# vaibhawvipul/taper

Hardware: AMD Instinct MI355X
Metric: MNIST samples/sec fwd+bwd+step (higher is better)
Workload: dtype f32; 1 GPU; mlp_784-128-10_b64; per_gpu_batch=64, global_batch=64, parallelism=single, comm=none, graph_record_steps=11577

## Files before the change

### include/taper_hip_debug.h

```cpp
#ifndef TAPER_HIP_DEBUG_H
#define TAPER_HIP_DEBUG_H

#include "taper_hip.h"

#ifdef __cplusplus
extern "C" {
#endif

int th_debug_mlp3_calls(int64_t *out);
int th_debug_mlp2_calls(int64_t *out);
int th_debug_mlp2_only(int which);
int th_debug_mlp2_ksplit(int ksplit);
int th_debug_set_chain_loop(int on);
int th_debug_chain_mlp3_only(int which);
int th_debug_set_chain_generic(int on);
int th_debug_last_conv_config(th_ctx *ctx, int *out6);
int th_debug_set_conv_img(th_ctx *ctx, int mode);
int th_debug_conv3x3_plan(int op, int n, int c_in, int h, int w, int c_out, int pad, int weight_layout, int relu_bias, int accumulate,
                          int w_misalign_bytes, int img_mode, int *out32);
int th_debug_qlinear_plan(int qtype, int batch, int in_features, int out_features, int x_misalign_bytes, int w_misalign_bytes, int *out8);
int th_debug_q8q8_plan(int batch, int in_features, int out_features, int *out4);
int th_debug_qconv_plan(int n, int c_in, int h, int w, int c_out, int k_h, int k_w, int s_h, int s_w, int pad_h, int pad_w, int *out8);
int th_debug_sgemm_plan(int trans_a, int trans_b, int m, int n, int k, int a_misalign_bytes, int b_misalign_bytes, int c_misalign_bytes, int *out12);
int th_debug_linear_fwd_ex_plan(int batch, int in_features, int out_features, int subtiles, int *out8);

int th_comm_debug_dump(th_comm *comm, th_ctx *ctx);
#ifdef __cplusplus
}
#endif

#endif
```

### taper_amd/csrc/common.h

```cpp
#pragma once

#include <hip/hip_runtime.h>

#include <cstdarg>
#include <cstdint>
#include <cstdio>
#include <array>
#include <atomic>
#include <map>
#include <string>
#include <unordered_map>
#include <unordered_set>
#include <vector>

#include "../../include/taper_hip.h"
#include "../../include/taper_hip_debug.h"

namespace th {

void set_error(const char *fmt, ...);

#define TH_HIP(expr)                                                                         \
    do {                                                                                     \
        hipError_t e_ = (expr);                                                              \
        if (e_ != hipSuccess) {                                                              \
            th::set_error("%s failed: %s (%s:%d)", #expr, hipGetErrorString(e_), __FILE__, __LINE__); \
            return 1;                                                                        \
        }                                                                                    \
    } while (0)

#define TH_REQUIRE(cond, ...)              \
    do {                                   \
        if (!(cond)) {                     \
            th::set_error(__VA_ARGS__);    \
            return 2;                      \
        }                                  \
    } while (0)

#define TH_SET_MAX_LDS(ctx_, fn_, bytes_)                                                                                \
    do {                                                                                                                 \
        static std::atomic<unsigned long long> th_lds_done_{0ull};                                                       \
        static std::atomic<int> th_lds_max_{0};                                                                          \
        const unsigned long long th_lds_bit_ = 1ull << ((ctx_)->device & 63);                                            \
        const int th_lds_want_ = (int)(bytes_);                                                                          \
        if (!(th_lds_done_.load(std::memory_order_relaxed) & th_lds_bit_) || th_lds_want_ > th_lds_max_.load(std::memory_order_relaxed)) { \
            TH_HIP(hipFuncSetAttribute((const void *)(fn_), hipFuncAttributeMaxDynamicSharedMemorySize, th_lds_want_));  \
            int th_lds_prev_ = th_lds_max_.load(std::memory_order_relaxed);                                              \
            if (th_lds_want_ > th_lds_prev_) {                                                                           \
                th_lds_max_.store(th_lds_want_, std::memory_order_relaxed);                                              \
                th_lds_done_.store(th_lds_bit_, std::memory_order_relaxed);    \
            } else {                                                                                                     \
                th_lds_done_.fetch_or(th_lds_bit_, std::memory_order_relaxed);                                           \
            }                                                                                                            \
        }                                                                                                                \
    } while (0)

#define TH_LAUNCH_CHECK() TH_HIP(hipGetLastError())

constexpr int kWave = 64;
constexpr int kNumCU = 256;
constexpr int kNumXCD = 8;

static inline int ceil_div(long a, long b) { return (int)((a + b - 1) / b); }

__device__ __forceinline__ void lds_barrier() {
    __builtin_amdgcn_fence(__ATOMIC_RELEASE, "workgroup", "local");
    __builtin_amdgcn_s_barrier();
    __builtin_amdgcn_fence(__ATOMIC_ACQUIRE, "workgroup", "local");
}

enum : int32_t { TH_DEVERR_NONE = 0, TH_DEVERR_TARGET_OOB = 1 };
static __device__ __attribute__((unused)) int32_t *g_err_word;
__device__ __forceinline__ void raise_target_oob(long cls, int classes) {
    int32_t *w = g_err_word;
    if (!w) return;
    w[1] = (int32_t)(cls > 0x7fffffffL ? 0x7fffffffL : cls);
    w[2] = classes;
    __threadfence_system();
    w[0] = TH_DEVERR_TARGET_OOB;
}
typedef int (*err_bind_fn)(int32_t *);
struct ErrBindReg { explicit ErrBindReg(err_bind_fn f); };
#define TH_USES_DEVICE_ERRORS()                                                                                        \
    namespace {                                                                                                        \
    int th_err_bind_here(int32_t *p) { return hipMemcpyToSymbol(HIP_SYMBOL(th::g_err_word), &p, sizeof(p)) == hipSuccess ? 0 : 1; } \
    th::ErrBindReg th_err_reg_here(th_err_bind_here);                                                                  \
    }

static inline int ew_grid(size_t n_items, int block) {
    long g = (long)((n_items + block - 1) / block);
    long cap = (long)kNumCU * 8;
    return (int)(g < 1 ? 1 : (g > cap ? cap : g));
}

}

struct th_ctx {
    int device = 0;
    hipStream_t stream = nullptr;
    std::multimap<size_t, void *> free_blocks;
    std::unordered_map<void *, size_t> block_size;
    std::unordered_set<void *> graph_owned;
    std::unordered_set<void *> graph_owned_freed;
    size_t bytes_reserved = 0, bytes_in_use = 0;
    bool capturing = false;
    std::vector<void *> capture_blocks;
    std::multimap<size_t, void *> capture_free;
    std::map<std::array<int, 8>, void *> conv_plans;
    int32_t *err_word = nullptr;
    int m2_max_ksplit = 8;
    bool fwd_subtiles = true;
    bool tail_split = true;
    const uint32_t *update_guard = nullptr;
    uint32_t *update_step_word = nullptr;
    unsigned *m2_arrive = nullptr;
};

struct th_graph {
    th_ctx *ctx = nullptr;
    hipGraph_t graph = nullptr;
    hipGraphExec_t exec = nullptr;
    std::vector<void *> blocks;
};

struct th_event {
    hipEvent_t ev = nullptr;
};
```

### taper_amd/csrc/fwd_tick.hip

```cpp
#include "small16_dev.h"

namespace th {

constexpr int kFwdAVec = 1, kFwdBVec = 2, kFwdXcd = 4;

struct FwdTickRest {
    float *C;
    const float *bias;
    int relu;
    int32_t *tick;
    AdamSlices x;
};

template <int NW, int RM, int RN>
__global__ __launch_bounds__(64 * NW) void sgemm_small16_tick(const float *X, const float *W, int m, int n, int k, int tile_rows, int grid_x,
                                                              int flags, FwdTickRest r) {
#ifdef TH_PROFILE
    __builtin_amdgcn_sched_barrier(0);
    const long long t_entry = wall_clock64();
    __builtin_amdgcn_sched_barrier(0);
#endif
    __shared__ float red[NW][64][4];
    if ((int)blockIdx.y < tile_rows) {
        int tm = blockIdx.y, tn = blockIdx.x;
        const int b = blockIdx.x + grid_x * blockIdx.y;
        if (flags & kFwdXcd) {
            constexpr int SBM = 32 / RM, SBN = 32 / RN;
            static_assert(SBN == 2 || SBN == 4, "sub-tiles of 16 or 8 columns");
            const int q = b & 7, j = b >> 3;
            tm = SBM * (q >> 2) + (j >> (SBN == 4 ? 2 : 1));
            tn = SBN * (q & 3) + (j & (SBN - 1));
        }
        const SmallArgs p{X, nullptr, W, r.C, nullptr, m, n, k, k, 1, 1, k, (k + 15) / 16 * 16, flags & kFwdAVec, flags & kFwdBVec,
                          Epilogue{1.0f, 0.0f, r.bias, r.relu, AdamDev{nullptr, nullptr, nullptr, nullptr, nullptr, 0.f, 0.f, 0.f, 0.f}, nullptr, nullptr}};
#ifdef TH_PROFILE
        small16_body<true, true, NW, false, RM, RN, true, true>(p, tm, tn, 0, red, t_entry, b);
#else
        small16_body<true, true, NW, false, RM, RN, false, true>(p, tm, tn, 0, red);
#endif
        return;
    }
    if (blockIdx.x == 0) adam_slices_then_tick(r.x, r.tick);
}

int fwd_tick_launch(th_ctx *ctx, const FwdTickLaunch &q, const float *d_x, const float *d_w, const float *d_b, float *d_y, int m, int n, int k,
                    int relu, const AdamSlices &x, int32_t *d_tick) {
    const FwdTickRest r{d_y, d_b, relu, d_tick, x};
    const int flags = (q.a_vec ? kFwdAVec : 0) | (q.b_vec ? kFwdBVec : 0) | (q.xcd_blocks ? kFwdXcd : 0);
    const dim3 grid(q.grid_x, q.grid_y, 1);
    const int tile_rows = q.grid_y - 1;
    if (q.rm == 8) hipLaunchKernelGGL((sgemm_small16_tick<16, 8, 8>), grid, dim3(1024), 0, ctx->stream, d_x, d_w, m, n, k, tile_rows, q.grid_x, flags, r);
    else if (q.waves == 16) hipLaunchKernelGGL((sgemm_small16_tick<16, 16, 16>), grid, dim3(1024), 0, ctx->stream, d_x, d_w, m, n, k, tile_rows, q.grid_x, flags, r);
    else hipLaunchKernelGGL((sgemm_small16_tick<4, 16, 16>), grid, dim3(256), 0, ctx->stream, d_x, d_w, m, n, k, tile_rows, q.grid_x, flags, r);
    TH_LAUNCH_CHECK();
    return 0;
}

}

#ifdef TH_PROFILE
extern "C" int th_debug_fwd_prof(th_ctx *ctx, long long *h_out, int n_blocks) {
    TH_REQUIRE(ctx && h_out && n_blocks >= 1 && n_blocks <= th::kFwdProfBlocks, "th_debug_fwd_prof: bad argument");
    TH_HIP(hipStreamSynchronize(ctx->stream));
    TH_HIP(hipMemcpyFromSymbol(h_out, HIP_SYMBOL(th::g_fwd_prof), (size_t)n_blocks * 2 * th::kFwdProfStamps * sizeof(long long)));
    return 0;
}
#endif
```

### taper_amd/csrc/gemm.hip

```cpp
#include "small16_dev.h"
#include "step_log_dev.h"

namespace th {

typedef float floatx16 __attribute__((ext_vector_type(16)));

static inline Epilogue make_ep(float alpha, float beta, const float *bias = nullptr, int relu = 0) {
    return Epilogue{alpha, beta, bias, relu, AdamDev{nullptr, nullptr, nullptr, nullptr, nullptr, 0.f, 0.f, 0.f, 0.f}, nullptr, nullptr};
}

__device__ __forceinline__ float epilogue_apply(float acc, float c_old, const Epilogue &ep, int col) {
    float v = ep.alpha * acc;
    if (ep.beta != 0.0f) v += ep.beta * c_old;
    if (ep.bias) v += ep.bias[col];
    if (ep.relu) v = v > 0.0f ? v : 0.0f;
    return v;
}

template <bool A_KC, bool B_KC, int NW>
__global__ __launch_bounds__(64 * NW) void sgemm_small16(SmallArgs p) {
    __shared__ float red[NW][64][4];
    small16_body<A_KC, B_KC, NW, false>(p, blockIdx.y, blockIdx.x, blockIdx.z, red);
}

// ... 749 lines not shown
    const long tiles = (long)pl.tiles_m * pl.tiles_n;
    pl.a_vec = a_kc && (a_bits & 15) == 0 && (a_rs % 4 == 0);
    pl.b_vec = b_kc && (b_bits & 15) == 0 && (b_cs % 4 == 0);
    int kz = 1;
    pl.waves = (tiles < 256 && k >= 256) ? 16 : 4;
    if (tiles < 64 && k >= 2048) {
        kz = (int)((256 + tiles - 1) / tiles);
        const int kz_max = k / 512;
        if (kz > kz_max) kz = kz_max;
        if (kz < 1) kz = 1;
    }
    if (k == 0) {
        pl.kslice = 16;
        pl.kz = 1;
        return;
    }
    int kslice = ceil_div(k, kz);
    kslice = (kslice + 15) / 16 * 16;
    pl.kslice = kslice;
    pl.kz = ceil_div(k, kslice);
}

static void plan_tile(GemmPlan &pl, int ts, int m, int n, int k, bool a_kc, bool b_kc, long lda, long ldb, uintptr_t a_bits, uintptr_t b_bits) {
    pl.tile = ts;
    pl.waves = 4;
    pl.tiles_m = ceil_div(m, ts);
    pl.tiles_n = ceil_div(n, ts);
    const int kz = ts == 128 ? tile128_kz(m, n, k) : tile64_kz(m, n, k);
    pl.kslice = ceil_div(ceil_div(k, kz), BK) * BK;
    pl.kz = ceil_div(k, pl.kslice);
    const bool vec = (a_bits & 15) == 0 && (b_bits & 15) == 0 && (lda % 4 == 0) && (ldb % 4 == 0) && ((a_kc ? k : m) % 4 == 0) &&
                     ((b_kc ? k : n) % 4 == 0) && m >= 4 && n >= 4 && k >= 4;
    const bool exact = (m % ts == 0) && (n % ts == 0) && (k % BK == 0) && vec && lda < (1L << 22) && ldb < (1L << 22);
    pl.a_vec = pl.b_vec = vec;
    pl.form = exact ? kFormExactDma : rag_dma(ts, a_kc, b_kc, k, vec, lda, ldb) ? kFormRagDma : vec ? kFormGuardVec : kFormGuardScalar;
    constexpr int kSliceXcdChunks = 14;
    pl.slice_xcd = pl.kz > 1 && pl.kslice >= kSliceXcdChunks * BK;
}

static GemmPlan gemm_plan(int trans_a, int trans_b, int m, int n, int k, uintptr_t a_bits, uintptr_t b_bits, uintptr_t c_bits) {
    const long a_rs = trans_a ? 1 : k, a_cs = trans_a ? m : 1;
    const long b_rs = trans_b ? 1 : n, b_cs = trans_b ? k : 1;
    const bool a_kc = !trans_a, b_kc = trans_b != 0;
    GemmPlan pl{};
    const TileClass tc = gemm_tile_class(m, n, k);
    if (tc == TileClass::Small) plan_small(pl, m, n, k, a_kc, b_kc, a_rs, b_cs, a_bits, b_bits);
    else plan_tile(pl, tc == TileClass::Tile128 ? 128 : 64, m, n, k, a_kc, b_kc, a_kc ? a_rs : a_cs, b_kc ? b_cs : b_rs, a_bits, b_bits);
    pl.reduce = pl.kz <= 1 ? kReduceNone : reduce_c_quad((long)m * n, c_bits) ? kReduceQuad : kReduceScalar;
    return pl;
}

int gemm_dispatch(th_ctx *ctx, int trans_a, int trans_b, int m, int n, int k, const float *A, const float *B, float *C,
                  const Epilogue &ep) {
    if (m == 0 || n == 0) return 0;
    const long a_rs = trans_a ? 1 : k, a_cs = trans_a ? m : 1;
    const long b_rs = trans_b ? 1 : n, b_cs = trans_b ? k : 1;
    const bool a_kc = !trans_a, b_kc = trans_b != 0;
    const GemmPlan pl = gemm_plan(trans_a, trans_b, m, n, k, (uintptr_t)A, (uintptr_t)B, (uintptr_t)C);
#define TH_GEMM_CASE(AK, BKC)                                                                         \
    if (a_kc == AK && b_kc == BKC)                                                                          \
        return pl.tile == 64  ? launch_tile<64, AK, BKC>(ctx, pl, A, B, C, m, n, k, a_rs, a_cs, b_rs, b_cs, ep) \
             : pl.tile == 128 ? launch_tile128<AK, BKC>(ctx, pl, A, B, C, m, n, k, a_rs, a_cs, b_rs, b_cs, ep)  \
                              : launch_small<AK, BKC>(ctx, pl, A, B, C, m, n, k, a_rs, a_cs, b_rs, b_cs, ep);
    TH_GEMM_CASE(true, true)
    TH_GEMM_CASE(true, false)
    TH_GEMM_CASE(false, true)
    TH_GEMM_CASE(false, false)
#undef TH_GEMM_CASE
    return 3;
}

int mlp3_grads_launch(th_ctx *ctx, const float *const dz[3], const float *const act[3], float *const dw[3], float *const db[3],
                      const int out_f[3], const int in_f[3], const th_adam_fuse *const wf[3], const th_adam_fuse *const bf[3], int batch,
                      const float *part, int n_blk, float *loss, float *ncorrect, float *metrics, int64_t capacity, int64_t *state,
                      int64_t advance, const float *gap_dx, const th_mlp3_gap *gap) {
    Mlp3GradArgs a{};
    int blocks = 0;
    for (int l = 0; l < 3; ++l) {
        LinearBwdArgs &q = a.job[l];
        const int tm = ceil_div(out_f[l], 16), tn = ceil_div(in_f[l], 16);
        q.dw_kz = 1;
        q.dw_tiles = dw[l] ? tm * tn : 0;
        q.n_dw = (q.dw_tiles + 7) & ~7;
        q.dw_tiles_m = tm;
        q.dw = SmallArgs{dz[l], nullptr, act[l], dw[l], nullptr, out_f[l], in_f[l], batch, 1, out_f[l], in_f[l], 1, (batch + 15) / 16 * 16, 0, 0,
                         make_ep(1.0f, 0.0f)};
        q.dw.ep.adam = make_adam_dev(dw[l] ? wf[l] : nullptr);
        q.db_adam = make_adam_dev(db[l] ? bf[l] : nullptr);
        q.dy = dz[l];
        q.db = db[l];
        q.batch = batch;
        q.out_f = out_f[l];
        q.n_db = db[l] ? ceil_div(out_f[l], 64) : 0;
        a.first[l] = blocks;
        blocks += q.n_dw + q.n_db;
    }
    a.first[3] = blocks;
    if (gap && gap->d_cnt) {
        a.gap_dx = gap_dx; a.gap_cnt = gap->d_cnt; a.gap_db = gap->d_gb; a.gap_c = in_f[0]; a.gap_hw = gap->hw;
        a.gap_adam = make_adam_dev(gap->b_fuse);
        blocks += ceil_div(a.gap_c, 16);
    }
    a.first[4] = blocks;
    a.part = part; a.n_blk = n_blk; a.batch = batch;
    a.loss = loss; a.ncorrect = ncorrect; a.metrics = metrics; a.capacity = capacity; a.state = state; a.advance = advance;
    hipLaunchKernelGGL(mlp3_grads_kernel, dim3(blocks + 1), dim3(256), 0, ctx->stream, a);
    TH_LAUNCH_CHECK();
    return 0;
}

int linear_fwd_partials(th_ctx *ctx, const float *x, const float *w, int m, int n, int k, float **partial_out, int *kz_out) {
    const int tiles_m = ceil_div(m, 16), tiles_n = ceil_div(n, 16);
    const long tiles = (long)tiles_m * tiles_n;
    SmallArgs p{x, nullptr, w, nullptr, nullptr, m, n, k, k, 1, 1, k, 0, 0, 0, make_ep(1.0f, 0.0f)};
    p.a_vec = aligned16(x) && (k % 4 == 0);
    p.b_vec = aligned16(w) && (k % 4 == 0);
    int kz = (int)std::min<long>((256 + tiles - 1) / tiles, k / 512);
    if (kz < 1) kz = 1;
    if (kz > 8) kz = 8;
    const int kslice = (ceil_div(k, kz) + 15) / 16 * 16;
    kz = ceil_div(k, kslice);
    p.kslice = kslice;
    void *ws = nullptr;
    if (th_malloc(ctx, (size_t)kz * m * n * sizeof(float), &ws)) return 1;
    p.partial = (float *)ws;
    if (tiles < 256 && k >= 256) hipLaunchKernelGGL((sgemm_small16<true, true, 16>), dim3(tiles_n, tiles_m, kz), dim3(1024), 0, ctx->stream, p);
    else hipLaunchKernelGGL((sgemm_small16<true, true, 4>), dim3(tiles_n, tiles_m, kz), dim3(256), 0, ctx->stream, p);
    TH_LAUNCH_CHECK();
    *partial_out = p.partial;
    *kz_out = kz;
    return 0;
}

struct FwdExPlan {
    int one_launch;
    int rm, rn;
    int waves;
    int grid_x, grid_y;
    int xcd_blocks;
};
static FwdExPlan fwd_ex_plan(int m, int n, int k, bool subtiles) {
    FwdExPlan pl{};
    const long tiles = (long)ceil_div(m, 16) * ceil_div(n, 16);
    if (!(m > 0 && n > 0 && k > 0 && !gemm_is_big(m, n, k) && !(tiles < 64 && k >= 2048))) return pl;
    pl.one_launch = 1;
    pl.rm = pl.rn = 16;
    pl.waves = (tiles < 256 && k >= 256) ? 16 : 4;
    if (subtiles && pl.waves == 16 && k <= 1024 && m <= 64 && n <= 128) pl.rm = pl.rn = 8;
    pl.grid_x = ceil_div(n, pl.rn);
    pl.grid_y = ceil_div(m, pl.rm) + 1;
    pl.xcd_blocks = pl.grid_x == 128 / pl.rn && pl.grid_y == 64 / pl.rm + 1;
    return pl;
}

}

using namespace th;

extern "C" {

#ifdef TH_PROFILE
int th_debug_gemm_prof(th_ctx *ctx, long long *h_out4) {
    TH_HIP(hipStreamSynchronize(ctx->stream));
    TH_HIP(hipMemcpyFromSymbol(h_out4, HIP_SYMBOL(th::g_gemm_prof), 4 * sizeof(long long)));
    return 0;
}
#endif

int th_sgemm(th_ctx *ctx, int trans_a, int trans_b, int m, int n, int k, float alpha, const float *d_a,
             const float *d_b, float beta, float *d_c) {
    TH_REQUIRE(ctx, "th_sgemm: null ctx");
    TH_REQUIRE(m >= 0 && n >= 0 && k >= 0, "th_sgemm: negative dimension");
    TH_REQUIRE((m == 0 || n == 0) || (d_c && (k == 0 || (d_a && d_b))), "th_sgemm: null device pointer");
    Epilogue ep = make_ep(alpha, beta);
    return gemm_dispatch(ctx, trans_a, trans_b, m, n, k, d_a, d_b, d_c, ep);
}

int th_debug_sgemm_plan(int trans_a, int trans_b, int m, int n, int k, int a_misalign_bytes, int b_misalign_bytes, int c_misalign_bytes, int *out12) {
    TH_REQUIRE(out12, "th_debug_sgemm_plan: null argument");
    TH_REQUIRE(m >= 1 && n >= 1 && k >= 0, "th_debug_sgemm_plan: bad shape m=%d n=%d k=%d", m, n, k);
    TH_REQUIRE(((a_misalign_bytes | b_misalign_bytes | c_misalign_bytes) & ~12) == 0,
               "th_debug_sgemm_plan: a float pointer lies 0, 4, 8 or 12 bytes off a 16-byte boundary (got %d %d %d)", a_misalign_bytes,
               b_misalign_bytes, c_misalign_bytes);
    const GemmPlan p = gemm_plan(trans_a != 0, trans_b != 0, m, n, k, (uintptr_t)a_misalign_bytes, (uintptr_t)b_misalign_bytes, (uintptr_t)c_misalign_bytes);
    const long wgs = (long)p.tiles_m * p.tiles_n * p.kz;
    const int out[12] = {p.tile, p.form, p.waves, p.a_vec, p.b_vec, p.kz, p.kslice, (int)std::min<long>(wgs, 0x7fffffff), p.slice_xcd, p.reduce,
                         p.tiles_m, p.tiles_n};
    std::copy(out, out + 12, out12);
    return 0;
}

int th_linear_fwd(th_ctx *ctx, const float *d_x, const float *d_w, const float *d_b, float *d_y, int batch,
                  int in_features, int out_features, int relu) {
    TH_REQUIRE(ctx && d_x && d_w && d_y, "th_linear_fwd: null argument");
    Epilogue ep = make_ep(1.0f, 0.0f, d_b, relu);
    return gemm_dispatch(ctx, 0, 1, batch, out_features, in_features, d_x, d_w, d_y, ep);
}

int th_linear_fwd_ex(th_ctx *ctx, const float *d_x, const float *d_w, const float *d_b, float *d_y, int batch, int in_features,
                     int out_features, int relu, const th_adam_slice *extra, int n_extra, int32_t *d_tick) {
    TH_REQUIRE(ctx && d_x && d_w && d_y, "th_linear_fwd_ex: null argument");
    TH_REQUIRE(n_extra >= 0 && n_extra <= TH_MAX_ADAM_SLICES && (n_extra == 0 || extra), "th_linear_fwd_ex: bad extra slices");
    for (int i = 0; i < n_extra; ++i)
        TH_REQUIRE(extra[i].f.d_p != d_w && extra[i].f.d_p != d_b, "th_linear_fwd_ex: a carried slice must not alias what this launch reads");
    const int m = batch, n = out_features, k = in_features;
    const FwdExPlan pl = fwd_ex_plan(m, n, k, ctx->fwd_subtiles != 0);
    if (pl.one_launch) {
        const FwdTickLaunch q{pl.rm, pl.waves, pl.grid_x, pl.grid_y, pl.xcd_blocks, aligned16(d_x) && (k % 4 == 0), aligned16(d_w) && (k % 4 == 0)};
        return fwd_tick_launch(ctx, q, d_x, d_w, d_b, d_y, m, n, k, relu, make_adam_slices(extra, n_extra, ctx), d_tick);
    }
    if (int rc = th_adam_slices(ctx, extra, n_extra)) return rc;
    if (d_tick)
        if (int rc = th_adam_tick(ctx, d_tick)) return rc;
    return th_linear_fwd(ctx, d_x, d_w, d_b, d_y, batch, in_features, out_features, relu);
}

int th_linear_fwd_ex_set_subtiles(th_ctx *ctx, int on) {
    TH_REQUIRE(ctx, "th_linear_fwd_ex_set_subtiles: null ctx");
    ctx->fwd_subtiles = on != 0;
    return 0;
}

int th_debug_linear_fwd_ex_plan(int batch, int in_features, int out_features, int subtiles, int *out8) {
    TH_REQUIRE(out8, "th_debug_linear_fwd_ex_plan: null argument");
    TH_REQUIRE(batch >= 1 && in_features >= 1 && out_features >= 1, "th_debug_linear_fwd_ex_plan: bad shape batch=%d in=%d out=%d", batch,
               in_features, out_features);
    const FwdExPlan pl = fwd_ex_plan(batch, out_features, in_features, subtiles != 0);
    const int out[8] = {pl.one_launch, pl.rm, pl.rn, pl.waves, 1, pl.grid_x, pl.grid_y, pl.xcd_blocks};
    std::copy(out, out + 8, out8);
    return 0;
}

}

namespace th {

constexpr int THIN_ROWS = 32;
__global__ __launch_bounds__(256) void linear_dx_thin_kernel(const float *__restrict__ dz, const float *__restrict__ w, const float *__restrict__ xmask,
                                                             float *__restrict__ dx, float *__restrict__ colpart, int batch, int in_f, int out_f,
                                                             int accumulate) {
    __shared__ float dzs[THIN_ROWS][16];
    const int t = threadIdx.x, r0 = blockIdx.y * THIN_ROWS, col = (blockIdx.x * 256 + t) * 4;
    for (int i = t; i < THIN_ROWS * 16; i += 256) {
        const int r = i >> 4, o = i & 15;
        dzs[r][o] = (r0 + r < batch && o < out_f) ? dz[(long)(r0 + r) * out_f + o] : 0.f;
    }
    float4 wv[16];
#pragma unroll
    for (int o = 0; o < 16; ++o) wv[o] = (o < out_f && col < in_f) ? *reinterpret_cast<const float4 *>(w + (long)o * in_f + col) : make_float4(0.f, 0.f, 0.f, 0.f);
    __syncthreads();
    if (col >= in_f) return;
    float4 cs = make_float4(0.f, 0.f, 0.f, 0.f);
#pragma unroll 8
    for (int r = 0; r < THIN_ROWS; ++r) {
        if (r0 + r >= batch) break;
        const long idx = (long)(r0 + r) * in_f + col;
        float4 v = accumulate ? *reinterpret_cast<const float4 *>(dx + idx) : make_float4(0.f, 0.f, 0.f, 0.f);
#pragma unroll
        for (int o = 0; o < 16; ++o) {
            const float d = dzs[r][o];
            v.x = fmaf(d, wv[o].x, v.x); v.y = fmaf(d, wv[o].y, v.y); v.z = fmaf(d, wv[o].z, v.z); v.w = fmaf(d, wv[o].w, v.w);
        }
        if (xmask) {
            const float4 m = *reinterpret_cast<const float4 *>(xmask + idx);
            v.x = m.x > 0.f ? v.x : 0.f; v.y = m.y > 0.f ? v.y : 0.f; v.z = m.z > 0.f ? v.z : 0.f; v.w = m.w > 0.f ? v.w : 0.f;
        }
        *reinterpret_cast<float4 *>(dx + idx) = v;
        cs.x += v.x; cs.y += v.y; cs.z += v.z; cs.w += v.w;
    }
    if (colpart) *reinterpret_cast<float4 *>(colpart + (long)blockIdx.y * in_f + col) = cs;
}

static int dx_epilogue_rows(int batch, int in_f, int out_f) {
    if (batch <= 0 || in_f <= 0 || out_f <= 0) return 0;
    if (out_f <= 16 && in_f % 4 == 0 && (long)batch * in_f >= (1L << 20)) return ceil_div(batch, THIN_ROWS);
    if (gemm_tile_class(batch, in_f, out_f) == TileClass::Tile128 && tile128_kz(batch, in_f, out_f) == 1) return ceil_div(batch, BM);
    return 0;
}

}

extern "C" {

int th_linear_bwd_dx_epilogue_rows(int batch, int in_features, int out_features) { return th::dx_epilogue_rows(batch, in_features, out_features); }

int th_linear_bwd_separate_products(int batch, int in_features, int out_features, int with_dx, int with_dw, int dx_epilogue) {
    const int ep_rows = (dx_epilogue && with_dx) ? th::dx_epilogue_rows(batch, in_features, out_features) : 0;
    const bool thin_dx = ep_rows > 0 && out_features <= 16;
    const bool dw_big = with_dw && gemm_is_big(out_features, in_features, batch);
    const bool dx_big = with_dx && !thin_dx && gemm_is_big(batch, in_features, out_features);
    return (!dw_big && !dx_big && batch <= 4096 && out_features <= 4096) ? 0 : 1;
}

int th_linear_bwd(th_ctx *ctx, const float *d_x, const float *d_w, const float *d_dy, const float *d_relu_y, float *d_dx,
                  float *d_dw, float *d_db, int batch, int in_features, int out_features, int accumulate_mask) {
    return th_linear_bwd_adam(ctx, d_x, d_w, d_dy, d_relu_y, d_dx, d_dw, d_db, batch, in_features, out_features, accumulate_mask,
                              nullptr, nullptr);
}

int th_linear_bwd_adam(th_ctx *ctx, const float *d_x, const float *d_w, const float *d_dy, const float *d_relu_y, float *d_dx,
                       float *d_dw, float *d_db, int batch, int in_features, int out_features, int accumulate_mask,
                       const th_adam_fuse *w_fuse, const th_adam_fuse *b_fuse) {
    return th_linear_bwd_adam_ex(ctx, d_x, d_w, d_dy, d_relu_y, d_dx, d_dw, d_db, batch, in_features, out_features, accumulate_mask,
                                 w_fuse, b_fuse, nullptr, 0);
}

int th_linear_bwd_adam_ex(th_ctx *ctx, const float *d_x, const float *d_w, const float *d_dy, const float *d_relu_y, float *d_dx,
                          float *d_dw, float *d_db, int batch, int in_features, int out_features, int accumulate_mask,
                          const th_adam_fuse *w_fuse, const th_adam_fuse *b_fuse, const th_adam_slice *extra, int n_extra) {
    return th_linear_bwd_adam_ex2(ctx, d_x, d_w, d_dy, d_relu_y, d_dx, d_dw, d_db, batch, in_features, out_features, accumulate_mask, w_fuse,
                                  b_fuse, extra, n_extra, 0, nullptr);
}

int th_linear_bwd_adam_ex2(th_ctx *ctx, const float *d_x, const float *d_w, const float *d_dy, const float *d_relu_y, float *d_dx,
                           float *d_dw, float *d_db, int batch, int in_features, int out_features, int accumulate_mask,
                           const th_adam_fuse *w_fuse, const th_adam_fuse *b_fuse, const th_adam_slice *extra, int n_extra, int mask_dx,
                           float *d_dx_colpart) {
    TH_REQUIRE(ctx && d_dy, "th_linear_bwd: null argument");
    const int ep_rows = (mask_dx || d_dx_colpart) ? th::dx_epilogue_rows(batch, in_features, out_features) : 0;
    TH_REQUIRE(!(mask_dx || d_dx_colpart) || (d_dx && d_x && ep_rows > 0 && !(accumulate_mask & 1)),
               "th_linear_bwd_adam_ex2: the dX epilogue (mask / column partials) needs d_dx written (not accumulated), d_x, and a shape "
               "th_linear_bwd_dx_epilogue_rows accepts (got %d x %d x %d)", batch, in_features, out_features);
    const bool thin_dx = ep_rows > 0 && out_features <= 16;
    TH_REQUIRE(n_extra >= 0 && n_extra <= TH_MAX_ADAM_SLICES && (n_extra == 0 || extra), "th_linear_bwd_adam_ex: bad extra slices");
    for (int i = 0; i < n_extra; ++i)
        TH_REQUIRE(extra[i].f.d_p != d_w || !d_dx, "th_linear_bwd_adam_ex: a carried slice must not alias the weight this launch reads");
    const AdamDev w_adam = make_adam_dev(d_dw ? w_fuse : nullptr), b_adam = make_adam_dev(d_db ? b_fuse : nullptr);
    TH_REQUIRE(!w_adam.p || !(accumulate_mask & 2), "th_linear_bwd_adam: a fused dW must not accumulate (grad slot must be None)");
    TH_REQUIRE(!b_adam.p || !(accumulate_mask & 4), "th_linear_bwd_adam: a fused db must not accumulate (grad slot must be None)");
    TH_REQUIRE(!d_dx || d_w, "th_linear_bwd: d_w required for d_dx");
    TH_REQUIRE(!d_dw || d_x, "th_linear_bwd: d_x required for d_dw");
    if (batch == 0 || out_features == 0 || in_features == 0) return th_adam_slices(ctx, extra, n_extra);
    if (thin_dx) {
        const float *dzt = d_dy;
        void *tmpz = nullptr;
        if (d_relu_y) {
            const size_t nz = (size_t)batch * out_features;
            if (th_malloc(ctx, nz * sizeof(float), &tmpz)) return 1;
            if (int rc = th_relu_bwd(ctx, d_relu_y, d_dy, (float *)tmpz, nz, 0)) {
                (void)th_free(ctx, tmpz);
                return rc;
            }
            dzt = (const float *)tmpz;
        }
        hipLaunchKernelGGL(th::linear_dx_thin_kernel, dim3(ceil_div(in_features, 1024), ceil_div(batch, th::THIN_ROWS)), dim3(256), 0, ctx->stream, dzt,
                           d_w, mask_dx ? d_x : nullptr, d_dx, d_dx_colpart, batch, in_features, out_features, 0);
        TH_LAUNCH_CHECK();
        if (tmpz && th_free(ctx, tmpz)) return 1;
        d_dx = nullptr;
    }
    const bool dw_big = d_dw && gemm_is_big(out_features, in_features, batch);
    const bool dx_big = d_dx && gemm_is_big(batch, in_features, out_features);
    if (!dw_big && !dx_big && batch <= 4096 && out_features <= 4096) {
        LinearBwdArgs q{};
        const int dw_tm = ceil_div(out_features, 16), dw_tn = ceil_div(in_features, 16);
        const int dx_tm = ceil_div(batch, 16), dx_tn = ceil_div(in_features, 16);
        int dw_kz = 1;
        if (d_dw && batch >= 512) dw_kz = batch / 256;
        q.dw_kz = dw_kz;
        q.dw_tiles = d_dw ? dw_tm * dw_tn * dw_kz : 0;
        q.n_dw = (q.dw_tiles + 7) & ~7;
        q.dw_tiles_m = dw_tm;
        q.n_dx = d_dx ? dx_tm * dx_tn : 0;
        q.dx_tiles_n = dx_tn;
        q.dw = SmallArgs{d_dy, d_relu_y, d_x, d_dw, nullptr, out_features, in_features, batch, 1, out_features, in_features, 1,
                         (batch + 15) / 16 * 16, 0, 0, make_ep(1.0f, (accumulate_mask & 2) ? 1.0f : 0.0f)};
        q.dx = SmallArgs{d_dy, d_relu_y, d_w, d_dx, nullptr, batch, in_features, out_features, out_features, 1, in_features, 1,
                         (out_features + 15) / 16 * 16, 0, 0, make_ep(1.0f, (accumulate_mask & 1) ? 1.0f : 0.0f)};
        q.dx.a_vec = aligned16(d_dy) && (!d_relu_y || aligned16(d_relu_y)) && (out_features % 4 == 0);
        const bool w_in_kernel = w_adam.p && !d_dx && dw_kz == 1;
        if (w_in_kernel) q.dw.ep.adam = w_adam;
        void *dw_part = nullptr;
// ... 69 lines not shown
```

### taper_amd/csrc/small16_dev.h

```cpp
#pragma once
#include "adam_dev.h"

namespace th {

typedef float floatx4 __attribute__((ext_vector_type(4)));

struct Epilogue {
    float alpha, beta;
    const float *bias;
    int relu;
    AdamDev adam;
    const float *mask;
    float *colpart;
};

struct SmallArgs {
    const float *A, *Amask, *B;
    float *C, *partial;
    int m, n, k;
    long a_rs, a_cs, b_rs, b_cs;
    int kslice, a_vec, b_vec;
    Epilogue ep;
    int xcd_blocks = 0;
};

struct FwdTickLaunch {
    int rm, waves, grid_x, grid_y, xcd_blocks;
    bool a_vec, b_vec;
};
int fwd_tick_launch(th_ctx *ctx, const FwdTickLaunch &q, const float *d_x, const float *d_w, const float *d_b, float *d_y, int m, int n, int k,
                    int relu, const AdamSlices &x, int32_t *d_tick);

#ifdef TH_PROFILE
constexpr int kFwdProfBlocks = 320;
constexpr int kFwdProfStamps = 8;
static __device__ __attribute__((unused)) long long g_fwd_prof[kFwdProfBlocks][2][kFwdProfStamps];
#define FWD_STAMP(i)                                                                          \
    do {                                                                                      \
        if constexpr (STAMPED) {                                                              \
            __builtin_amdgcn_sched_barrier(0);                                                \
            if (stamp_slot >= 0) g_fwd_prof[stamp_blk][stamp_slot][i] = wall_clock64();       \
            __builtin_amdgcn_sched_barrier(0);                                                \
        }                                                                                     \
    } while (0)
#define FWD_LANDED(v) do { if constexpr (STAMPED) asm volatile("" ::"v"(v)); } while (0)
#else
#define FWD_STAMP(i) do { } while (0)
#define FWD_LANDED(v) do { } while (0)
#endif

#define SMALL16_REQUEST_EPILOGUE()                                                    \
    do {                                                                              \
        if (e_ok) {                                                                   \
            if (p.ep.beta != 0.0f && !p.partial) e_cold = p.C[e_ix];                  \
            if (fuse_adam) {                                                          \
                e_p = p.ep.adam.p[e_ix];                                              \
                e_m = p.ep.adam.m[e_ix];                                              \
                e_v = p.ep.adam.v[e_ix];                                              \
                e_step = adam_dev_step(p.ep.adam);                                    \
            }                                                                         \
            if (p.ep.bias) e_bias = p.ep.bias[ecol];                                  \
        }                                                                             \
    } while (0)
template <bool A_KC, bool B_KC, int NW, bool MASKED, int RM = 16, int RN = 16, bool STAMPED = false, bool EP_LATE = false>
__device__ __forceinline__ void small16_body(const SmallArgs &p, int tile_row, int tile_col, int zslice, float (*red)[64][4],
                                             long long stamp_entry = 0, int stamp_blk_arg = -1) {
    constexpr bool SUB = RM < 16 || RN < 16;
    const int lane = threadIdx.x & 63, wave = threadIdx.x >> 6;
    const int r = lane & 15, g = lane >> 4;
    const int row0 = tile_row * RM, col0 = tile_col * RN;
    const int kbeg_slice = zslice * p.kslice;
    const int kend_slice = min(p.k, kbeg_slice + p.kslice);
    const int kwave = ((kend_slice - kbeg_slice + 16 * NW - 1) / (16 * NW)) * 16;
    const int kbeg = kbeg_slice + wave * kwave;
    const int kend = min(kend_slice, kbeg + kwave);
#ifdef TH_PROFILE
    const int stamp_blk = stamp_blk_arg >= 0 ? stamp_blk_arg : blockIdx.x + gridDim.x * blockIdx.y;
    const int stamp_last = max((kend_slice - kbeg_slice) / kwave - 1, 0) % NW;
    const int stamp_slot = (lane != 0 || stamp_blk >= kFwdProfBlocks) ? -1 : wave == 0 ? 0 : wave == stamp_last ? 1 : -1;
    if constexpr (STAMPED)
        if (stamp_slot >= 0) g_fwd_prof[stamp_blk][stamp_slot][6] = stamp_entry;
#endif
    FWD_STAMP(0);

    const int arow = row0 + (SUB ? r & (RM - 1) : r), bcol = col0 + (SUB ? r & (RN - 1) : r);
    const bool a_ok = (!SUB || r < RM) && arow < p.m, b_ok = (!SUB || r < RN) && bcol < p.n;
    const long a_off = (long)(a_ok ? arow : SUB ? row0 : 0) * p.a_rs;
    const float *ap = p.A + a_off;
    const float *mp = MASKED ? p.Amask + a_off : nullptr;
    const float *bp = p.B + (long)(b_ok ? bcol : SUB ? col0 : 0) * p.b_cs;

    const int ecol = col0 + (lane & 15);
    const bool fuse_adam = p.ep.adam.p != nullptr && p.partial == nullptr;
    const int erow = row0 + (lane >> 4) * 4 + wave;
    const bool e_sub = !SUB || ((lane >> 4) * 4 + wave < RM && (lane & 15) < RN);
    const bool e_ok = wave < 4 && erow < p.m && ecol < p.n && e_sub;
    const long e_ix = e_ok ? (long)erow * p.n + ecol : 0;
    float e_bias = 0.f, e_cold = 0.f, e_p = 0.f, e_m = 0.f, e_v = 0.f, e_step = 0.f;
    if constexpr (!EP_LATE) {
        SMALL16_REQUEST_EPILOGUE();
    }
    constexpr int CH = 4;
    floatx4 acc = {0.f, 0.f, 0.f, 0.f};
    for (int kk0 = kbeg; kk0 < kend; kk0 += 16 * CH) {
        float av[CH][4], bv[CH][4];
#pragma unroll
        for (int c = 0; c < CH; ++c) {
            const int kb = kk0 + 16 * c + g * 4;
            if (A_KC && p.a_vec && kb + 4 <= kend) {
                float4 t = *reinterpret_cast<const float4 *>(ap + kb);
                av[c][0] = t.x; av[c][1] = t.y; av[c][2] = t.z; av[c][3] = t.w;
                if (MASKED) {
                    float4 q = *reinterpret_cast<const float4 *>(mp + kb);
                    av[c][0] = q.x > 0.f ? av[c][0] : 0.f; av[c][1] = q.y > 0.f ? av[c][1] : 0.f;
                    av[c][2] = q.z > 0.f ? av[c][2] : 0.f; av[c][3] = q.w > 0.f ? av[c][3] : 0.f;
                }
            } else {
#pragma unroll
                for (int s = 0; s < 4; ++s) {
                    const bool in = kb + s < kend;
                    float v = in ? ap[(long)(kb + s) * p.a_cs] : 0.f;
                    if (MASKED) v = (in && mp[(long)(kb + s) * p.a_cs] > 0.f) ? v : 0.f;
                    av[c][s] = v;
                }
            }
            if (B_KC && p.b_vec && kb + 4 <= kend) {
                float4 t = *reinterpret_cast<const float4 *>(bp + kb);
                bv[c][0] = t.x; bv[c][1] = t.y; bv[c][2] = t.z; bv[c][3] = t.w;
            } else {
#pragma unroll
                for (int s = 0; s < 4; ++s) bv[c][s] = (kb + s < kend) ? bp[(long)(kb + s) * p.b_rs] : 0.f;
            }
        }
        if (kk0 == kbeg) {
            FWD_STAMP(1);
            FWD_LANDED(av[0][0]);
            FWD_LANDED(bv[0][0]);
            FWD_STAMP(2);
        }
        if constexpr (EP_LATE) {
            if (kk0 == kbeg) SMALL16_REQUEST_EPILOGUE();
        }
#pragma unroll
        for (int c = 0; c < CH; ++c) {
            if (kk0 + 16 * c >= kend) break;
#pragma unroll
            for (int s = 0; s < 4; ++s) {
                const float a = a_ok ? av[c][s] : 0.f;
                const float b = b_ok ? bv[c][s] : 0.f;
                acc = __builtin_amdgcn_mfma_f32_16x16x4f32(a, b, acc, 0, 0, 0);
            }
        }
    }
    if constexpr (EP_LATE) {
        if (kbeg >= kend) SMALL16_REQUEST_EPILOGUE();
    }
    FWD_LANDED(acc[0]);
    FWD_STAMP(3);

    if (!SUB || (g * 4 < RM && r < RN)) {
#pragma unroll
        for (int i = 0; i < 4; ++i) red[wave][lane][i] = acc[i];
    }
    __syncthreads();
    FWD_STAMP(4);
    if (wave < 4 && e_sub) {
        float sum = red[0][lane][wave];
        for (int w = 1; w < NW; ++w) sum += red[w][lane][wave];
        if (e_ok) {
            if (p.partial) {
                p.partial[(long)zslice * p.m * p.n + e_ix] = sum;
            } else {
                float out = p.ep.alpha * sum;
                if (p.ep.beta != 0.0f) out += p.ep.beta * e_cold;
                if (p.ep.bias) out += e_bias;
                if (p.ep.relu) out = out > 0.0f ? out : 0.0f;
                p.C[e_ix] = out;
                if (fuse_adam) {
                    const AdamDev &ad = p.ep.adam;
                    const AdamMV x = adam_moments(ad, e_p, e_m, e_v, out);
                    ad.m[e_ix] = x.m;
                    ad.v[e_ix] = x.v;
                    ad.p[e_ix] = adam_param(ad, e_p, x, e_step);
                }
            }
        }
    }
#ifdef TH_PROFILE
    if constexpr (STAMPED) __builtin_amdgcn_s_waitcnt(0x0F70);
#endif
    FWD_STAMP(5);
}

}
```

Measured before the change: 6.041 million samples/s.

## Stack X and W rows into one MFMA operand in small forward tile kernel

```diff
diff --git a/experiments/cu_intake.hip b/experiments/cu_intake.hip
--- /dev/null
+++ b/experiments/cu_intake.hip
@@ -0,0 +1,150 @@
+#include <hip/hip_runtime.h>
+#include <algorithm>
+#include <cmath>
+#include <cstdio>
+#include <cstring>
+#include <vector>
+
+#define CK(x) do { hipError_t e_ = (x); if (e_ != hipSuccess) { printf("%s: %s\n", #x, hipGetErrorString(e_)); return 1; } } while (0)
+
+typedef float floatx4 __attribute__((ext_vector_type(4)));
+constexpr int M = 64, N = 128, K = 784, NW = 16, KW = 64;
+enum { ALIASED, MASKED, STACKED, NOLOAD };
+
+__host__ __device__ inline float fill_value(unsigned i, unsigned salt) {
+    unsigned h = (i + salt) * 2654435761u;
+    h ^= h >> 15;
+    return (float)(int)(h & 0xffff) * (1.0f / 32768.0f) - 1.0f;
+}
+__global__ __launch_bounds__(256) void rewrite(float4 *xw, int quads, unsigned salt) {
+    const int q = blockIdx.x * 256 + threadIdx.x;
+    if (q < quads) xw[q] = make_float4(fill_value(4 * q, salt), fill_value(4 * q + 1, salt), fill_value(4 * q + 2, salt), fill_value(4 * q + 3, salt));
+}
+
+template <int F>
+__global__ __launch_bounds__(64 * NW) void k1_shaped(const float *__restrict__ X, const float *__restrict__ W, float *__restrict__ H) {
+    __shared__ float red[NW][64][4];
+    const int lane = threadIdx.x & 63, wave = __builtin_amdgcn_readfirstlane(threadIdx.x >> 6);
+    const int r = lane & 15, g = lane >> 4;
+    const int row0 = blockIdx.y * 8, col0 = blockIdx.x * 8;
+    const int kbeg = wave * KW, kend = min(K, kbeg + KW);
+    const bool low = r < 8;
+    float av[4][4] = {}, bv[4][4] = {};
+    if (F == ALIASED || F == MASKED) {
+        const float *ap = X + (long)(row0 + (r & 7)) * K, *bp = W + (long)(col0 + (r & 7)) * K;
+        if (F == ALIASED || low) {
+#pragma unroll
+            for (int c = 0; c < 4; ++c) {
+                if (kbeg + 16 * c >= kend) break;
+                const float4 t = *reinterpret_cast<const float4 *>(ap + kbeg + 16 * c + 4 * g);
+                const float4 u = *reinterpret_cast<const float4 *>(bp + kbeg + 16 * c + 4 * g);
+                av[c][0] = t.x; av[c][1] = t.y; av[c][2] = t.z; av[c][3] = t.w;
+                bv[c][0] = u.x; bv[c][1] = u.y; bv[c][2] = u.z; bv[c][3] = u.w;
+            }
+        }
+    } else if (F == STACKED) {
+        const float *sp = low ? X + (long)(row0 + r) * K : W + (long)(col0 + r - 8) * K;
+#pragma unroll
+        for (int c = 0; c < 4; ++c) {
+            if (kbeg + 16 * c >= kend) break;
+            const float4 t = *reinterpret_cast<const float4 *>(sp + kbeg + 16 * c + 4 * g);
+            av[c][0] = t.x; av[c][1] = t.y; av[c][2] = t.z; av[c][3] = t.w;
+        }
+    } else {
+#pragma unroll
+        for (int c = 0; c < 4; ++c)
+#pragma unroll
+            for (int s = 0; s < 4; ++s) av[c][s] = bv[c][s] = (float)(lane + 4 * c + s + wave) * 0.001f;
+    }
+    floatx4 acc = {0.f, 0.f, 0.f, 0.f};
+#pragma unroll
+    for (int c = 0; c < 4; ++c) {
+        if (kbeg + 16 * c >= kend) break;
+#pragma unroll
+        for (int s = 0; s < 4; ++s) {
+            if (F == STACKED) acc = __builtin_amdgcn_mfma_f32_16x16x4f32(av[c][s], av[c][s], acc, 0, 0, 0);
+            else acc = __builtin_amdgcn_mfma_f32_16x16x4f32(low ? av[c][s] : 0.f, low ? bv[c][s] : 0.f, acc, 0, 0, 0);
+        }
+    }
+    const int c_off = F == STACKED ? 8 : 0;
+    const bool mine = g < 2 && r >= c_off && r < c_off + 8;
+    if (mine) {
+#pragma unroll
+        for (int i = 0; i < 4; ++i) red[wave][lane][i] = acc[i];
+    }
+    __syncthreads();
+    if (wave < 4 && mine) {
+        float sum = red[0][lane][wave];
+        for (int w = 1; w < NW; ++w) sum += red[w][lane][wave];
+        H[(long)(row0 + 4 * g + wave) * N + col0 + r - c_off] = sum;
+    }
+}
+
+template <int F>
+static double pair_us(hipStream_t s, float *xw, float *h) {
+    const int pairs = 100, reps = 20, quads = (M + N) * K / 4;
+    const float *x = xw, *w = xw + (size_t)M * K;
+    hipGraph_t g; hipGraphExec_t ge;
+    (void)hipStreamBeginCapture(s, hipStreamCaptureModeGlobal);
+    for (int i = 0; i < pairs; ++i) {
+        hipLaunchKernelGGL(rewrite, dim3((quads + 255) / 256), dim3(256), 0, s, (float4 *)xw, quads, 17u);
+        hipLaunchKernelGGL(k1_shaped<F>, dim3(N / 8, M / 8), dim3(64 * NW), 0, s, x, w, h);
+    }
+    (void)hipStreamEndCapture(s, &g);
+    (void)hipGraphInstantiate(&ge, g, nullptr, nullptr, 0);
+    for (int i = 0; i < 3; ++i) (void)hipGraphLaunch(ge, s);
+    (void)hipStreamSynchronize(s);
+    hipEvent_t e0, e1; (void)hipEventCreate(&e0); (void)hipEventCreate(&e1);
+    (void)hipEventRecord(e0, s);
+    for (int i = 0; i < reps; ++i) (void)hipGraphLaunch(ge, s);
+    (void)hipEventRecord(e1, s);
+    (void)hipEventSynchronize(e1);
+    float ms = 0; (void)hipEventElapsedTime(&ms, e0, e1);
+    (void)hipEventDestroy(e0); (void)hipEventDestroy(e1);
+    (void)hipGraphExecDestroy(ge); (void)hipGraphDestroy(g);
+    return ms * 1e3 / (reps * pairs);
+}
+
+int main() {
+    hipStream_t s; CK(hipStreamCreate(&s));
+    float *xw, *h[4];
+    CK(hipMalloc(&xw, (size_t)(M + N) * K * sizeof(float)));
+    for (auto &p : h) { CK(hipMalloc(&p, (size_t)M * N * sizeof(float))); CK(hipMemset(p, 0, (size_t)M * N * sizeof(float))); }
+    const int rounds = 5;
+    double us[4][rounds];
+    for (int i = 0; i < rounds; ++i) {
+        us[ALIASED][i] = pair_us<ALIASED>(s, xw, h[ALIASED]);
+        us[MASKED][i] = pair_us<MASKED>(s, xw, h[MASKED]);
+        us[STACKED][i] = pair_us<STACKED>(s, xw, h[STACKED]);
+        us[NOLOAD][i] = pair_us<NOLOAD>(s, xw, h[NOLOAD]);
+    }
+    CK(hipGetLastError());
+    CK(hipStreamSynchronize(s));
+
+    std::vector<float> out[3], hx((size_t)(M + N) * K);
+    for (int f = 0; f < 3; ++f) { out[f].resize((size_t)M * N); CK(hipMemcpy(out[f].data(), h[f], out[f].size() * sizeof(float), hipMemcpyDeviceToHost)); }
+    for (size_t i = 0; i < hx.size(); ++i) hx[i] = fill_value((unsigned)i, 17u);
+    double worst = 0;
+    for (int i = 0; i < M; ++i)
+        for (int j = 0; j < N; ++j) {
+            double ref = 0;
+            for (int k = 0; k < K; ++k) ref += (double)hx[(size_t)i * K + k] * hx[(size_t)(M + j) * K + k];
+            worst = std::max(worst, std::fabs(ref - out[ALIASED][(size_t)i * N + j]));
+        }
+    const int diff_b = memcmp(out[ALIASED].data(), out[MASKED].data(), out[0].size() * sizeof(float)) != 0;
+    const int diff_c = memcmp(out[ALIASED].data(), out[STACKED].data(), out[0].size() * sizeof(float)) != 0;
+    printf("H of (a) against the float64 product: worst |error| %.3g; (b) %s (a), (c) %s (a) bit for bit\n", worst, diff_b ? "DIFFERS from" : "equals",
+           diff_c ? "DIFFERS from" : "equals");
+
+    const char *name[4] = {"(a) aliased, 8 loads", "(b) masked,  8 loads", "(c) stacked, 4 loads", "(d) no operand loads"};
+    double med[4];
+    printf("rewrite + K1-shaped launch, %d rounds in turn: us per pair\n", rounds);
+    for (int f = 0; f < 4; ++f) {
+        std::sort(us[f], us[f] + rounds);
+        med[f] = us[f][rounds / 2];
+        printf("  %s: median %6.3f  (%6.3f .. %6.3f, spread %5.3f)\n", name[f], med[f], us[f][0], us[f][rounds - 1], us[f][rounds - 1] - us[f][0]);
+    }
+    printf("  (a) - (d) %6.3f   (b) - (d) %6.3f   (c) - (d) %6.3f   (a) - (c) %6.3f\n", med[ALIASED] - med[NOLOAD], med[MASKED] - med[NOLOAD],
+           med[STACKED] - med[NOLOAD], med[ALIASED] - med[STACKED]);
+    return (diff_b || diff_c || worst > 1e-2) ? 2 : 0;
+}
diff --git a/include/taper_hip_debug.h b/include/taper_hip_debug.h
--- a/include/taper_hip_debug.h
+++ b/include/taper_hip_debug.h
@@ -23,6 +23,9 @@
 int th_debug_qconv_plan(int n, int c_in, int h, int w, int c_out, int k_h, int k_w, int s_h, int s_w, int pad_h, int pad_w, int *out8);
 int th_debug_sgemm_plan(int trans_a, int trans_b, int m, int n, int k, int a_misalign_bytes, int b_misalign_bytes, int c_misalign_bytes, int *out12);
 int th_debug_linear_fwd_ex_plan(int batch, int in_features, int out_features, int subtiles, int *out8);
+int th_debug_linear_fwd_ex_set_stacked(th_ctx *ctx, int on);
+int th_debug_linear_fwd_ex_stacked(int batch, int in_features, int out_features, int subtiles, int stacking, int x_misalign_bytes,
+                                   int w_misalign_bytes, int *out1);
 
 int th_comm_debug_dump(th_comm *comm, th_ctx *ctx);
 #ifdef __cplusplus
diff --git a/taper_amd/csrc/common.h b/taper_amd/csrc/common.h
--- a/taper_amd/csrc/common.h
+++ b/taper_amd/csrc/common.h
@@ -110,6 +110,7 @@
     int32_t *err_word = nullptr;
     int m2_max_ksplit = 8;
     bool fwd_subtiles = true;
+    bool fwd_stacked = true;
     bool tail_split = true;
     const uint32_t *update_guard = nullptr;
     uint32_t *update_step_word = nullptr;
diff --git a/taper_amd/csrc/fwd_tick.hip b/taper_amd/csrc/fwd_tick.hip
--- a/taper_amd/csrc/fwd_tick.hip
+++ b/taper_amd/csrc/fwd_tick.hip
@@ -12,14 +12,16 @@
     AdamSlices x;
 };
 
-template <int NW, int RM, int RN>
+template <int NW, int RM, int RN, bool STACKED = false>
 __global__ __launch_bounds__(64 * NW) void sgemm_small16_tick(const float *X, const float *W, int m, int n, int k, int tile_rows, int grid_x,
                                                               int flags, FwdTickRest r) {
+    static_assert(!STACKED || (RM == 8 && RN == 8), "the stacked operand holds 8 rows of X and 8 of W");
 #ifdef TH_PROFILE
     __builtin_amdgcn_sched_barrier(0);
     const long long t_entry = wall_clock64();
     __builtin_amdgcn_sched_barrier(0);
 #endif
+    if constexpr (STACKED) asm volatile("" ::"s"(X), "s"(W), "s"(m), "s"(n), "s"(k), "s"(tile_rows), "s"(grid_x), "s"(flags));
     __shared__ float red[NW][64][4];
     if ((int)blockIdx.y < tile_rows) {
         int tm = blockIdx.y, tn = blockIdx.x;
@@ -34,9 +36,11 @@
         const SmallArgs p{X, nullptr, W, r.C, nullptr, m, n, k, k, 1, 1, k, (k + 15) / 16 * 16, flags & kFwdAVec, flags & kFwdBVec,
                           Epilogue{1.0f, 0.0f, r.bias, r.relu, AdamDev{nullptr, nullptr, nullptr, nullptr, nullptr, 0.f, 0.f, 0.f, 0.f}, nullptr, nullptr}};
 #ifdef TH_PROFILE
-        small16_body<true, true, NW, false, RM, RN, true, true>(p, tm, tn, 0, red, t_entry, b);
+        if constexpr (STACKED) small16_stacked_body<NW, true>(p, tm, tn, red, t_entry, b);
+        else small16_body<true, true, NW, false, RM, RN, true, true>(p, tm, tn, 0, red, t_entry, b);
 #else
-        small16_body<true, true, NW, false, RM, RN, false, true>(p, tm, tn, 0, red);
+        if constexpr (STACKED) small16_stacked_body<NW>(p, tm, tn, red);
+        else small16_body<true, true, NW, false, RM, RN, false, true>(p, tm, tn, 0, red);
 #endif
         return;
     }
@@ -49,7 +53,8 @@
     const int flags = (q.a_vec ? kFwdAVec : 0) | (q.b_vec ? kFwdBVec : 0) | (q.xcd_blocks ? kFwdXcd : 0);
     const dim3 grid(q.grid_x, q.grid_y, 1);
     const int tile_rows = q.grid_y - 1;
-    if (q.rm == 8) hipLaunchKernelGGL((sgemm_small16_tick<16, 8, 8>), grid, dim3(1024), 0, ctx->stream, d_x, d_w, m, n, k, tile_rows, q.grid_x, flags, r);
+    if (q.stacked) hipLaunchKernelGGL((sgemm_small16_tick<16, 8, 8, true>), grid, dim3(1024), 0, ctx->stream, d_x, d_w, m, n, k, tile_rows, q.grid_x, flags, r);
+    else if (q.rm == 8) hipLaunchKernelGGL((sgemm_small16_tick<16, 8, 8>), grid, dim3(1024), 0, ctx->stream, d_x, d_w, m, n, k, tile_rows, q.grid_x, flags, r);
     else if (q.waves == 16) hipLaunchKernelGGL((sgemm_small16_tick<16, 16, 16>), grid, dim3(1024), 0, ctx->stream, d_x, d_w, m, n, k, tile_rows, q.grid_x, flags, r);
     else hipLaunchKernelGGL((sgemm_small16_tick<4, 16, 16>), grid, dim3(256), 0, ctx->stream, d_x, d_w, m, n, k, tile_rows, q.grid_x, flags, r);
     TH_LAUNCH_CHECK();
diff --git a/taper_amd/csrc/gemm.hip b/taper_amd/csrc/gemm.hip
--- a/taper_amd/csrc/gemm.hip
+++ b/taper_amd/csrc/gemm.hip
@@ -925,6 +925,9 @@
     pl.xcd_blocks = pl.grid_x == 128 / pl.rn && pl.grid_y == 64 / pl.rm + 1;
     return pl;
 }
+static bool fwd_ex_stacked(const FwdExPlan &pl, bool stacking, bool x_vec, bool w_vec) {
+    return stacking && pl.one_launch && pl.rm == 8 && pl.rn == 8 && pl.waves == 16 && x_vec && w_vec;
+}
 
 }
 
@@ -979,7 +982,8 @@
     const int m = batch, n = out_features, k = in_features;
     const FwdExPlan pl = fwd_ex_plan(m, n, k, ctx->fwd_subtiles != 0);
     if (pl.one_launch) {
-        const FwdTickLaunch q{pl.rm, pl.waves, pl.grid_x, pl.grid_y, pl.xcd_blocks, aligned16(d_x) && (k % 4 == 0), aligned16(d_w) && (k % 4 == 0)};
+        const bool x_vec = aligned16(d_x) && (k % 4 == 0), w_vec = aligned16(d_w) && (k % 4 == 0);
+        const FwdTickLaunch q{pl.rm, pl.waves, pl.grid_x, pl.grid_y, pl.xcd_blocks, x_vec, w_vec, fwd_ex_stacked(pl, ctx->fwd_stacked, x_vec, w_vec)};
         return fwd_tick_launch(ctx, q, d_x, d_w, d_b, d_y, m, n, k, relu, make_adam_slices(extra, n_extra, ctx), d_tick);
     }
     if (int rc = th_adam_slices(ctx, extra, n_extra)) return rc;
@@ -991,6 +995,26 @@
 int th_linear_fwd_ex_set_subtiles(th_ctx *ctx, int on) {
     TH_REQUIRE(ctx, "th_linear_fwd_ex_set_subtiles: null ctx");
     ctx->fwd_subtiles = on != 0;
+    return 0;
+}
+
+int th_debug_linear_fwd_ex_set_stacked(th_ctx *ctx, int on) {
+    TH_REQUIRE(ctx, "th_debug_linear_fwd_ex_set_stacked: null ctx");
+    ctx->fwd_stacked = on != 0;
+    return 0;
+}
+
+int th_debug_linear_fwd_ex_stacked(int batch, int in_features, int out_features, int subtiles, int stacking, int x_misalign_bytes,
+                                   int w_misalign_bytes, int *out1) {
+    TH_REQUIRE(out1, "th_debug_linear_fwd_ex_stacked: null argument");
+    TH_REQUIRE(batch >= 1 && in_features >= 1 && out_features >= 1, "th_debug_linear_fwd_ex_stacked: bad shape batch=%d in=%d out=%d", batch,
+               in_features, out_features);
+    TH_REQUIRE(((x_misalign_bytes | w_misalign_bytes) & ~12) == 0,
+               "th_debug_linear_fwd_ex_stacked: a float pointer lies 0, 4, 8 or 12 bytes off a 16-byte boundary (got %d %d)", x_misalign_bytes,
+               w_misalign_bytes);
+    const FwdExPlan pl = fwd_ex_plan(batch, out_features, in_features, subtiles != 0);
+    const bool k4 = in_features % 4 == 0;
+    *out1 = fwd_ex_stacked(pl, stacking != 0, x_misalign_bytes == 0 && k4, w_misalign_bytes == 0 && k4);
     return 0;
 }
 
diff --git a/taper_amd/csrc/small16_dev.h b/taper_amd/csrc/small16_dev.h
--- a/taper_amd/csrc/small16_dev.h
+++ b/taper_amd/csrc/small16_dev.h
@@ -27,6 +27,7 @@
 struct FwdTickLaunch {
     int rm, waves, grid_x, grid_y, xcd_blocks;
     bool a_vec, b_vec;
+    bool stacked;
 };
 int fwd_tick_launch(th_ctx *ctx, const FwdTickLaunch &q, const float *d_x, const float *d_w, const float *d_b, float *d_y, int m, int n, int k,
                     int relu, const AdamSlices &x, int32_t *d_tick);
@@ -192,4 +193,87 @@
     FWD_STAMP(5);
 }
 
+template <int NW, bool STAMPED = false>
+__device__ __forceinline__ void small16_stacked_body(const SmallArgs &p, int tile_row, int tile_col, float (*red)[64][4],
+                                                     long long stamp_entry = 0, int stamp_blk_arg = -1) {
+    const int lane = threadIdx.x & 63, wave = __builtin_amdgcn_readfirstlane(threadIdx.x >> 6);
+    const int r = lane & 15, g = lane >> 4;
+    const int row0 = tile_row * 8, col0 = tile_col * 8;
+    const int kwave = ((p.k + 16 * NW - 1) / (16 * NW)) * 16;
+    const int kbeg = wave * kwave;
+    const int kend = min(p.k, kbeg + kwave);
+#ifdef TH_PROFILE
+    const int stamp_blk = stamp_blk_arg >= 0 ? stamp_blk_arg : blockIdx.x + gridDim.x * blockIdx.y;
+    const int stamp_last = max(p.k / kwave - 1, 0) % NW;
+    const int stamp_slot = (lane != 0 || stamp_blk >= kFwdProfBlocks) ? -1 : wave == 0 ? 0 : wave == stamp_last ? 1 : -1;
+    if constexpr (STAMPED)
+        if (stamp_slot >= 0) g_fwd_prof[stamp_blk][stamp_slot][6] = stamp_entry;
+#endif
+    FWD_STAMP(0);
+
+    const bool is_x = r < 8;
+    const int srow = is_x ? row0 + r : col0 + r - 8;
+    const bool s_ok = srow < (is_x ? p.m : p.n);
+    const float *sp = (is_x ? p.A : p.B) + (long)(s_ok ? srow : is_x ? row0 : col0) * p.k;
+
+    const int ecol = col0 + (lane & 15) - 8;
+    const int erow = row0 + (lane >> 4) * 4 + wave;
+    const bool e_sub = (lane >> 4) * 4 + wave < 8 && (lane & 15) >= 8;
+    const bool e_ok = wave < 4 && erow < p.m && ecol < p.n && e_sub;
+    const long e_ix = e_ok ? (long)erow * p.n + ecol : 0;
+    float e_bias = 0.f;
+    constexpr int CH = 4;
+    floatx4 acc = {0.f, 0.f, 0.f, 0.f};
+    for (int kk0 = kbeg; kk0 < kend; kk0 += 16 * CH) {
+        float sv[CH][4];
+        bool in[CH];
+#pragma unroll
+        for (int c = 0; c < CH; ++c) {
+            const int kb = kk0 + 16 * c + g * 4;
+            in[c] = kb + 4 <= kend;
+            const float4 t = kk0 + 16 * c < kend ? *reinterpret_cast<const float4 *>(sp + (in[c] ? kb : kk0)) : float4{0.f, 0.f, 0.f, 0.f};
+            sv[c][0] = t.x; sv[c][1] = t.y; sv[c][2] = t.z; sv[c][3] = t.w;
+        }
+        if (kk0 == kbeg) {
+            FWD_STAMP(1);
+            FWD_LANDED(sv[0][0]);
+            FWD_STAMP(2);
+            if (e_ok && p.ep.bias) e_bias = p.ep.bias[ecol];
+        }
+#pragma unroll
+        for (int c = 0; c < CH; ++c) {
+            if (kk0 + 16 * c >= kend) break;
+#pragma unroll
+            for (int s = 0; s < 4; ++s) {
+                const float v = s_ok && in[c] ? sv[c][s] : 0.f;
+                acc = __builtin_amdgcn_mfma_f32_16x16x4f32(v, v, acc, 0, 0, 0);
+            }
+        }
+    }
+    if (kbeg >= kend && e_ok && p.ep.bias) e_bias = p.ep.bias[ecol];
+    FWD_LANDED(acc[0]);
+    FWD_STAMP(3);
+
+    if (g < 2 && r >= 8) {
+#pragma unroll
+        for (int i = 0; i < 4; ++i) red[wave][lane][i] = acc[i];
+    }
+    __syncthreads();
+    FWD_STAMP(4);
+    if (wave < 4 && e_sub) {
+        float sum = red[0][lane][wave];
+        for (int w = 1; w < NW; ++w) sum += red[w][lane][wave];
+        if (e_ok) {
+            float out = p.ep.alpha * sum;
+            if (p.ep.bias) out += e_bias;
+            if (p.ep.relu) out = out > 0.0f ? out : 0.0f;
+            p.C[e_ix] = out;
+        }
+    }
+#ifdef TH_PROFILE
+    if constexpr (STAMPED) __builtin_amdgcn_s_waitcnt(0x0F70);
+#endif
+    FWD_STAMP(5);
 }
+
+}
```

Result: no change. 6.000 million samples/s (-0.7%).
